# gabrielspmoreira/chameleon_recsys

Hardware: NVIDIA H100
Metric: NAR train interactions/sec (higher is better)
Workload: dtype f32 (wgmma: bf16x3 (error-compensated) forward, single-pass TF32 backward; fp32 accumulate)

## Files before the change

chameleon_recsys_b200/_lib.py:

```python
from __future__ import annotations

import ctypes as C
import os
from typing import Optional

HERE = os.path.dirname(os.path.abspath(__file__))
LIB_PATH = os.path.join(HERE, 'libnar_b200.so')

NAR_MAX_SEGMENTS = 24
NAR_MAX_SRC = 16
NAR_MAX_COLS = 1024

ACT_NONE, ACT_LEAKY, ACT_TANH = 0, 1, 2


class NarError(RuntimeError):
    pass


class Segment(C.Structure):
    _fields_ = [('kind', C.c_int32), ('col', C.c_int32), ('width', C.c_int32), ('card', C.c_int32),
                ('src', C.c_int32), ('ld', C.c_int32), ('table', C.c_void_p), ('grad', C.c_void_p)]


# ... 117 lines not shown
    'nar_dropout_rows': (C.c_int, [vp, vp, i64, i64, i64, vp, i64, i64, i64, C.c_int, f32, u64, u32, vp]),
    'nar_rank_candidates': (C.c_int, [vp, vp, i64, i64, i32, vp, vp, vp, vp]),
    'nar_car_combine_grid': (C.c_int, [vp, vp, i64, i64, i64, C.c_int, vp, vp]),
    'nar_topn_candidates': (C.c_int, [vp, vp, i64, i64, i32, vp, vp, i64, vp, vp, vp, vp]),
    'nar_engine_recommend_workspace_bytes': (C.c_int, [vp, i64, i64, i64, i32, i64, C.POINTER(i64), C.POINTER(i64),
                                                       C.POINTER(i64)]),
    'nar_engine_recommend': (C.c_int, [vp, C.POINTER(StepIO), vp, vp, i64, vp, i64, i32, i32, i64, i64, vp, vp, vp, vp]),
    'nar_host_state_update': (C.c_int, [vp, i64, vp, vp, i64, i64, vp, vp, vp, vp, i64, C.c_double]),
    'nar_host_state_update_batch': (C.c_int, [vp, i64, vp, vp, vp, i64, i64, i64, vp, vp, vp, vp, vp, i64, C.c_double]),
    'nar_state_update': (C.c_int, [vp, vp, i64, vp, vp, i64, i64, i64, vp, vp, vp, vp, vp, vp, i64, C.c_double, vp, vp]),
    'nar_colsum_add': (C.c_int, [vp, i64, i64, i64, vp, vp]),
    'nar_act_bwd': (C.c_int, [vp, vp, i64, C.c_int, vp, vp]),
    'nar_l2_loss_add': (C.c_int, [vp, i64, f32, vp, vp]),
    'nar_transpose_f32': (C.c_int, [vp, i64, i64, i64, vp, i64, vp]),
    'nar_adam_tf': (C.c_int, [vp, vp, vp, vp, i64, i64, f32, f32, f32, f32, f32, i64, vp, vp]),
    'nar_tf32_lo': (C.c_int, [vp, i64, vp, vp]),
    'nar_baselines_clear': (C.c_int, [vp, vp, vp, vp, i64, vp]),
    'nar_baselines_rehash': (C.c_int, [vp, vp, vp, vp, i64, vp, vp, vp, vp, i64, vp, vp]),
    'nar_baselines_update': (C.c_int, [vp, vp, vp, vp, i64, vp, vp, i64, i64, i64, i32, i64, vp, vp]),
    'nar_baselines_buffer_hist': (C.c_int, [vp, i64, i64, vp, vp, vp, vp]),
    'nar_baselines_row_norms': (C.c_int, [vp, i64, i64, i64, vp, vp]),
    'nar_baselines_score': (C.c_int, [vp, vp, vp, vp, i64, vp, vp, vp, i64, i64, i64, vp, vp, vp, vp, i64, i64, vp, i64,
                                      C.c_double, C.c_double, i32, i32, vp, vp, vp, vp, vp]),
    'nar_sknn_update': (C.c_int, [vp, vp, vp, i64, i64, i64, i64, vp, vp, vp, vp, vp, i64, i64, i64, vp, vp]),
    'nar_sknn_score': (C.c_int, [vp, vp, vp, i64, i64, i64, i64, vp, vp, vp, i64, i64, i64, i64, i64, i64, i32, i32, i32,
                                 vp, vp, vp, vp, vp]),
    'nar_eval_metrics_mark': (C.c_int, [vp, i64, i64, i32, vp, vp, vp]),
    'nar_eval_metrics_lists': (C.c_int, [vp, i64, i64, i64, i64, i64, i64, i32, vp, i64, vp, vp, i64, i64, vp, i64,
                                         C.c_double, vp, vp, vp, vp]),
    'nar_eval_metrics_reduce': (C.c_int, [vp, i64, i64, i64, vp, vp]),
# ... 55 lines not shown
```

chameleon_recsys_b200/csrc/engine.cu:

```cuda
#include "common.cuh"
#include <string.h>
#include <stdio.h>
#include <stdlib.h>

extern "C" int nar_sample_negatives_uidx(nar_ctx*, const int64_t*, int64_t, int64_t, int64_t, int64_t, const int64_t*, int64_t,
                                         int64_t, int64_t, uint64_t, uint32_t, int64_t*, int32_t*, const int64_t**,
                                         const int32_t**, void*, int64_t, void*);
namespace nar {
int recommend_rows(const int32_t* pos_idx, int64_t L, const int64_t* item_clicked, const int64_t* cand_ids, int64_t N,
                   int32_t* row_pos, int64_t* row_item, cudaStream_t st);
}

namespace {

constexpr int N_EVENTS = 64;

inline int64_t align_up(int64_t x, int64_t a) { return (x + a - 1) / a * a; }

struct Carver {
  char* base; int64_t off;
  explicit Carver(void* b) : base(static_cast<char*>(b)), off(0) {}
  template <typename T> T* take(int64_t n) {
    T* p = base ? reinterpret_cast<T*>(base + off) : nullptr;
    off = align_up(off + (n > 0 ? n : 1) * (int64_t)sizeof(T), 256);
    return p;
  }
};

struct PrepBufs {
  void* sampler_ws; int64_t sampler_bytes;
  int64_t* neg; int32_t* neg_uidx; float* stats; int32_t* row_pos; int64_t* row_item;
  int32_t* base_pos; int64_t* base_item; int64_t U;
};

struct StepBufs {
  float *X, *dX, *H1, *E, *dE, *dH1, *F1, *PR, *logits, *PD, *dPD, *Z1, *Z2, *Z3, *dZ1, *dZ2, *dZ3, *dPR, *dF1, *dHO;
  float *GX[NAR_MAX_LAYERS], *HO[NAR_MAX_LAYERS], *GT[NAR_MAX_LAYERS], *CD[NAR_MAX_LAYERS], *dGX[NAR_MAX_LAYERS],
        *HPV[NAR_MAX_LAYERS], *dHOb[NAR_MAX_LAYERS], *HOd[NAR_MAX_LAYERS],
        *UO[NAR_MAX_LAYERS], *RH[NAR_MAX_LAYERS];
  float *PP, *PI, *PC, *DB;
  float* H1cT; int64_t ldr;
};

}

constexpr int MAX_PLANES = 32;
struct PlaneSet {
// ... 2 lines not shown
  int64_t dst[MAX_PLANES];
  const float* W[MAX_PLANES]; void* out[MAX_PLANES];
  uint16_t* buf; void* descs;
};

struct nar_engine {
  nar_ctx* ctx;
  nar_model_cfg cfg;
  PlaneSet planes;
  cudaStream_t aux;
  cudaEvent_t ev[N_EVENTS];
  int ev_i;
  float* WhT[NAR_MAX_LAYERS];
  int64_t launches;
  int fused_product;
};

namespace {

bool fused_product(const nar_engine* e) {
  const nar_model_cfg& c = e->cfg;
  return e->fused_product && c.ranking == 0 && c.K + 1 <= 128 && c.fwd_precision == 4 && c.bwd_precision == 1;
}

int64_t gate_blocks(const nar_model_cfg& c) { return c.rnn_cell == NAR_CELL_LSTM ? 4 : c.rnn_cell == NAR_CELL_GRU ? 3 : 2; }

nar_feature_plan call_plan(const nar_model_cfg& c, const nar_step_io* io, const float* stats) {
  nar_feature_plan plan = c.plan;
  for (int i = 0; i < NAR_MAX_SRC; ++i) { plan.ctx_int[i] = io->ctx_int[i]; plan.ctx_float[i] = io->ctx_float[i]; }
  plan.pop_norm = io->pop_norm;
// ... 5 lines not shown
  const nar_model_cfg& c = e->cfg;
  const int64_t K = c.K, n_cand = K + 1, Rcap = L_cap * (n_cand + 1);
  Carver cv(base);
  int64_t sb = 0;
  nar_sample_negatives_workspace(Bg, T + 1, c.buf_len, K, &sb);
  pb->sampler_bytes = sb;
  pb->sampler_ws = cv.take<char>(sb);
  pb->neg = cv.take<int64_t>(Bg * T * K);
  pb->neg_uidx = cv.take<int32_t>(c.dedup ? Bg * T * K : 1);
  pb->stats = cv.take<float>(24);
  pb->row_pos = cv.take<int32_t>(Rcap);
  pb->row_item = cv.take<int64_t>(Rcap);
  pb->U = K * 20 + 1;
  pb->base_pos = cv.take<int32_t>(c.dedup ? 2 * L_cap + pb->U : 1);
  pb->base_item = cv.take<int64_t>(c.dedup ? 2 * L_cap + pb->U : 1);
  (void)B;
  return cv.off;
}

void session_carve(const nar_model_cfg& c, int64_t L, Carver& cv, StepBufs* sb) {
  const int64_t Hp = c.Hp;
  for (int i = 0; i < c.layers; ++i) {
    sb->GX[i] = cv.take<float>(L * gate_blocks(c) * Hp); sb->HO[i] = cv.take<float>(L * Hp);
    if (c.rnn_cell != NAR_CELL_LSTM) sb->GT[i] = cv.take<float>(L * Hp);
    sb->CD[i] = cv.take<float>(L * Hp);
    if (c.rnn_cell == NAR_CELL_GRU) { sb->UO[i] = cv.take<float>(L * Hp); sb->RH[i] = cv.take<float>(L * Hp); }
  }
  sb->F1 = cv.take<float>(L * 512);
  sb->PR = cv.take<float>(L * c.C);
}
// ... 175 lines not shown
  }
  s.fwd(rnn_in, Hp, c.off_W3, 512, c.off_b3, sb.F1, 512, L, 512, Hp, NAR_ACT_LEAKY_RELU, st);
  if (drop) s.dropout(sb.F1, sb.F1, L, 512, io->pos_idx, 4, st);
  s.fwd(sb.F1, 512, c.off_W4, C, c.off_b4, sb.PR, C, L, C, 512, NAR_ACT_TANH, st);
}

int run_step(nar_engine* e, const nar_step_io* io, cudaStream_t main) {
  const nar_model_cfg& c = e->cfg;
  const int64_t B = io->B, T = io->T, L = io->L, K = c.K, n_cand = K + 1, Rc = L * n_cand, R = L + Rc;
  const int64_t C = c.C, Hp = c.Hp, Fp = c.Fp, c0 = c.ctx_col0;
  const int train = io->train;
  if (L > io->L_cap || L < 0 || B <= 0) return NAR_ERR_INVALID;
  PrepBufs pb; StepBufs sb;
  if (prep_carve(e, io->Bg, B, T, io->L_cap, io->prep_ws, &pb) > io->prep_ws_bytes) return NAR_ERR_WORKSPACE;
  if (step_carve(e, io->L_cap, train, io->ws, &sb) > io->ws_bytes) return NAR_ERR_WORKSPACE;
  NAR_CHECK_CUDA(cudaMemsetAsync(io->loss, 0, 4 * sizeof(float), main));
  if (train) NAR_CHECK_CUDA(cudaMemsetAsync(c.grads, 0, (size_t)c.n_params * sizeof(float), main));
  if (L == 0) return NAR_OK;
  const bool drop = train && c.keep_prob < 1.f;
  if (drop && c.dedup) return NAR_ERR_INVALID;
  Seq s(e, io, main);
  const float inv_count = 1.0f / (float)(io->L_global > 0 ? io->L_global : 1);
  const int64_t U = pb.U, NB = 2 * L + U;

  const nar_feature_plan plan = call_plan(c, io, pb.stats);
  nar_row_layout rl;
  if (c.dedup) { rl.n_rows = NB; rl.n_input = L; rl.n_cand = 0; rl.n_positive = L; rl.n_full = 2 * L; rl.ctx_col0 = c0; }
  else { rl.n_rows = R; rl.n_input = L; rl.n_cand = n_cand; rl.n_positive = 0; rl.n_full = R; rl.ctx_col0 = c0; }
  const int32_t* g_pos = c.dedup ? pb.base_pos : pb.row_pos;
  const int64_t* g_item = c.dedup ? pb.base_item : pb.row_item;
  s.chk(nar_gather_features(e->ctx, &plan, g_pos, g_item, &rl, io->event_ts, io->max_ts, sb.X, main));
  if (drop) s.dropout(sb.X, sb.X, R, Fp, pb.row_pos, 0, main);

  float* H1c = sb.H1 + L * C; float* Ec = sb.E + L * C;
  clicked_rows_forward(s, sb, L, drop);
  if (c.dedup) {
    s.fwd(sb.X + L * Fp, Fp, c.off_W1, C, c.off_b1, sb.PP, C, L, C, Fp, NAR_ACT_NONE, main);
    s.fwd(sb.X + 2 * L * Fp, Fp, c.off_W1, C, -1, sb.PI, C, U, C, c0, NAR_ACT_NONE, main);
    s.fwd(sb.X + c0, Fp, c.off_W1 + c0 * C, C, c.off_b1, sb.PC, C, L, C, Fp - c0, NAR_ACT_NONE, main);
    s.chk(nar_car_combine_t(sb.PP, sb.PC, sb.PI, io->pos_idx, pb.neg_uidx, L, K, C, NAR_ACT_LEAKY_RELU, sb.H1cT, sb.ldr, main));
    s.fwd(sb.H1cT, sb.ldr, c.off_W2, C, c.off_b2, Ec, C, Rc, C, C, NAR_ACT_TANH, main, nullptr, 0, 0, 0);
  } else {
    s.fwd(sb.X + L * Fp, Fp, c.off_W1, C, c.off_b1, H1c, C, Rc, C, Fp, NAR_ACT_LEAKY_RELU, main);
    s.fwd(H1c, C, c.off_W2, C, c.off_b2, Ec, C, Rc, C, C, NAR_ACT_TANH, main);
  }
  s.join();

  nar_novelty_reg nov; memset(&nov, 0, sizeof(nov));
  nov.factor = c.novelty_reg_factor; nov.log_base = c.plan.log_base_novelty; nov.pop_norm = io->pop_norm;
  nov.cand_ids = pb.row_item + L; nov.loss_nov = io->loss + 2;
  const nar_novelty_reg* novp = c.novelty_reg_factor > 0.f ? &nov : nullptr;
  const bool fused = fused_product(e);
  s.scorer(Ec, sb.PR, L, n_cand, fused, sb.PD, sb.Z1, sb.Z2, sb.Z3, sb.logits, io->loss, inv_count, train ? sb.dZ3 : nullptr,
           train ? sb.dE + L * C : nullptr, train ? sb.dPR : nullptr, novp);
  if (c.reg_l2 > 0.f && c.rank == 0) { cudaStream_t st = s.fork(); s.chk(nar_l2_loss_add(c.params, c.reg_end, c.reg_l2, io->loss + 1, st)); }
  if (!train || s.rc) { s.join(); return s.rc; }

  float* dEc = sb.dE + L * C;
  if (c.ranking == 0) {
    { cudaStream_t st = s.fork(); s.wgrad(sb.Z2, 64, sb.dZ3, 32, c.off_M[2], c.ld_M[2], 64, 32, Rc, st); s.bgrad(sb.dZ3, 32, Rc, 32, c.off_c[2], st); }
    s.dgrad(sb.dZ3, 32, c.off_M[2], c.ld_M[2], sb.dZ2, 64, Rc, 64, 32, NAR_ACT_LEAKY_RELU, sb.Z2, 64, 0, main);
    { cudaStream_t st = s.fork(); s.wgrad(sb.Z1, 128, sb.dZ2, 64, c.off_M[1], c.ld_M[1], 128, 64, Rc, st); s.bgrad(sb.dZ2, 64, Rc, 64, c.off_c[1], st); }
    s.dgrad(sb.dZ2, 64, c.off_M[1], c.ld_M[1], sb.dZ1, 128, Rc, 128, 64, NAR_ACT_LEAKY_RELU, sb.Z1, 128, 0, main);
    {
      cudaStream_t st = s.fork();
      if (fused) s.wgrad(Ec, C, sb.dZ1, 128, c.off_M[0], c.ld_M[0], C, 128, Rc, st, sb.PR, C, n_cand);
      else s.wgrad(sb.PD, C, sb.dZ1, 128, c.off_M[0], c.ld_M[0], C, 128, Rc, st);
      s.bgrad(sb.dZ1, 128, Rc, 128, c.off_c[0], st);
    }
    if (fused) {
// ... 220 lines not shown
  add(c.off_M[0], C, 128, c.ld_M[0]); add(c.off_M[1], 128, 64, c.ld_M[1]); add(c.off_M[2], 64, 32, c.ld_M[2]);
  for (int i = 0; i < c.layers; ++i) {
    const int64_t gw = gate_blocks(c) * Hp;
    add(c.off_Wx[i], i == 0 ? C : Hp, gw, gw);
  }
  if (overflow) return NAR_ERR_INVALID;
  if (!ps.buf) {
    cudaMalloc(&ps.buf, (size_t)total * sizeof(uint16_t));
    cudaMemset(ps.buf, 0, (size_t)total * sizeof(uint16_t));
    cudaMalloc(&ps.descs, MAX_PLANES * 32);
  }
  for (int i = 0; i < ps.n; ++i) { ps.W[i] = c.params + ps.off_W[i]; ps.out[i] = ps.buf + ps.dst[i]; }
  return NAR_OK;
}

int planes_refresh(nar_engine* e, cudaStream_t st) {
  PlaneSet& ps = e->planes;
  if (!ps.buf || ps.n == 0) return NAR_ERR_INVALID;
  ++e->launches;
  return nar_pack_bf16x3(ps.W, ps.out, ps.K, ps.N, ps.ldw, ps.ld_out, ps.n, ps.descs, st);
}

extern "C" int nar_engine_create(nar_ctx* ctx, const nar_model_cfg* cfg, nar_engine** out) {
  if (!ctx || !cfg || !out) return NAR_ERR_INVALID;
  *out = nullptr;
  if (cfg->layers < 1 || cfg->layers > NAR_MAX_LAYERS || cfg->rnn_cell < NAR_CELL_UGRNN || cfg->rnn_cell > NAR_CELL_LSTM ||
      cfg->ranking < 0 || cfg->ranking > 1)
    return NAR_ERR_UNSUPPORTED;
  if ((cfg->C & 3) || (cfg->Hp & 3) || (cfg->Fp & 3) || (cfg->ctx_col0 & 3) || cfg->ctx_col0 <= 0 || cfg->ctx_col0 >= cfg->Fp)
    return NAR_ERR_INVALID;
  if (!cfg->params || !cfg->grads || !cfg->adam_m || !cfg->adam_v || !cfg->params_lo) return NAR_ERR_INVALID;
  nar_engine* e = new nar_engine();
  memset(e, 0, sizeof(*e));
  e->ctx = ctx; e->cfg = *cfg;
  { const char* v = getenv("NAR_FUSED_SCORER_PRODUCT"); e->fused_product = !(v && atoi(v) == 0); }
  NAR_CHECK_CUDA(cudaSetDevice(ctx->device));
  if (cudaStreamCreateWithFlags(&e->aux, cudaStreamNonBlocking) != cudaSuccess) { delete e; return NAR_ERR_NO_DEVICE; }
  for (int i = 0; i < N_EVENTS; ++i)
    if (cudaEventCreateWithFlags(&e->ev[i], cudaEventDisableTiming) != cudaSuccess) { delete e; return NAR_ERR_NO_DEVICE; }
  for (int i = 0; i < cfg->layers; ++i) {
    const size_t wht = (size_t)gate_blocks(*cfg) * cfg->Hp * cfg->Hp;
    if (cudaMalloc(&e->WhT[i], wht * sizeof(float)) != cudaSuccess) { delete e; return NAR_ERR_NO_DEVICE; }
  }
  if (planes_build(e) != NAR_OK) { delete e; return NAR_ERR_INVALID; }
  if (!e->planes.buf || !e->planes.descs) { delete e; return NAR_ERR_NO_DEVICE; }
  *out = e;
  return NAR_OK;
}

extern "C" int nar_engine_refresh(nar_engine* e, void* stream) {
  if (!e) return NAR_ERR_INVALID;
  return planes_refresh(e, as_stream(stream));
}

extern "C" int nar_engine_destroy(nar_engine* e) {
  if (!e) return NAR_OK;
  cudaStreamSynchronize(e->aux);
  for (int i = 0; i < NAR_MAX_LAYERS; ++i) if (e->WhT[i]) cudaFree(e->WhT[i]);
  for (int i = 0; i < N_EVENTS; ++i) if (e->ev[i]) cudaEventDestroy(e->ev[i]);
  if (e->aux) cudaStreamDestroy(e->aux);
  if (e->planes.buf) cudaFree(e->planes.buf);
  if (e->planes.descs) cudaFree(e->planes.descs);
  delete e;
  return NAR_OK;
}

extern "C" int nar_engine_update_cfg(nar_engine* e, const nar_model_cfg* cfg) {
  if (!e || !cfg) return NAR_ERR_INVALID;
  if (cfg->layers != e->cfg.layers || cfg->Hp != e->cfg.Hp || cfg->C != e->cfg.C || cfg->Fp != e->cfg.Fp ||
      cfg->rnn_cell != e->cfg.rnn_cell) return NAR_ERR_INVALID;
  e->cfg = *cfg;
  return planes_build(e);
}

extern "C" int nar_engine_workspace_bytes(const nar_engine* e, int64_t Bg, int64_t B, int64_t T, int64_t L_cap, int32_t train,
                                          int64_t* prep_bytes, int64_t* ws_bytes) {
  if (!e || Bg <= 0 || B <= 0 || T <= 0 || L_cap < 0) return NAR_ERR_INVALID;
  PrepBufs pb; StepBufs sb;
  if (prep_bytes) *prep_bytes = prep_carve(e, Bg, B, T, L_cap, nullptr, &pb);
  if (ws_bytes) *ws_bytes = step_carve(e, L_cap, train, nullptr, &sb);
  return NAR_OK;
}

extern "C" int nar_engine_prepare(nar_engine* e, const nar_step_io* io, void* stream) {
  if (!e || !io || !io->prep_ws || !io->all_items || !io->buffer) return NAR_ERR_INVALID;
  const nar_model_cfg& c = e->cfg;
  const int64_t B = io->B, Bg = io->Bg, T = io->T, L = io->L, K = c.K, n_cand = K + 1, R = L + L * n_cand;
  if (L > io->L_cap || io->sess0 < 0 || io->sess0 + B > Bg) return NAR_ERR_INVALID;
  PrepBufs pb;
  if (prep_carve(e, Bg, B, T, io->L_cap, io->prep_ws, &pb) > io->prep_ws_bytes) return NAR_ERR_WORKSPACE;
  cudaStream_t st = as_stream(stream);
  int64_t* neg_local = pb.neg + io->sess0 * T * K;
  int32_t* uidx_local = c.dedup ? pb.neg_uidx + io->sess0 * T * K : nullptr;
  const int64_t* uitems = nullptr; const int32_t* n_unique = nullptr;
  int rc = nar_sample_negatives_uidx(e->ctx, io->all_items, Bg, T + 1, io->sess0, B, io->buffer, c.buf_len, K, c.n_from_buffer,
                                     c.sampler_seed, io->sampler_step, neg_local, uidx_local, &uitems, &n_unique, pb.sampler_ws,
                                     pb.sampler_bytes, st);
  e->launches += 2;
  if (rc) return rc;
  if (L <= 0) return NAR_OK;
  rc = nar_build_rows(io->pos_idx, L, io->item_clicked, io->label_next, pb.neg, K, pb.row_pos, pb.row_item, st);
  ++e->launches;
  if (rc) return rc;
  rc = nar_feature_stats(e->ctx, io->buffer, c.buf_len, c.n_norm, c.plan.created_at_ts, io->pop_norm, io->max_ts,
                         c.plan.log_base_recency, c.plan.log_base_novelty, pb.row_pos, pb.row_item, R, L, n_cand, io->event_ts,
                         pb.stats, st);
  ++e->launches;
  if (rc) return rc;
  if (c.dedup) {
    rc = nar_build_base_rows(io->pos_idx, L, io->item_clicked, io->label_next, uitems, n_unique, pb.U, pb.neg_uidx, K, pb.base_pos,
                             pb.base_item, st);
    ++e->launches;
  }
  return rc;
}

extern "C" int nar_engine_step(nar_engine* e, const nar_step_io* io, void* stream) {
  if (!e || !io || !io->prep_ws || !io->ws || !io->loss) return NAR_ERR_INVALID;
  return run_step(e, io, as_stream(stream));
}

extern "C" int nar_engine_apply(nar_engine* e, const nar_step_io* io, void* stream) {
  if (!e || !io) return NAR_ERR_INVALID;
  const nar_model_cfg& c = e->cfg;
  ++e->launches;
  int rc = nar_adam_tf(c.params, c.grads, c.adam_m, c.adam_v, c.n_params, c.reg_end, c.reg_l2, c.lr, c.beta1, c.beta2, c.eps,
                       io->global_step + 1, c.params_lo, stream);
  if (rc == NAR_OK && c.fwd_precision == 4) rc = planes_refresh(e, as_stream(stream));
  return rc;
}

extern "C" int nar_engine_recommend_workspace_bytes(const nar_engine* e, int64_t L, int64_t Q, int64_t N, int32_t gather_q,
                                                    int64_t budget_bytes, int64_t* ws_bytes, int64_t* q_block, int64_t* n_block) {
  if (!e || !ws_bytes || !q_block || !n_block || L <= 0 || Q <= 0 || Q > L || N <= 0) return NAR_ERR_INVALID;
  const int64_t b = rec_plan(e, L, Q, N, gather_q != 0, budget_bytes, q_block, n_block);
  if (b < 0) return NAR_ERR_WORKSPACE;
  *ws_bytes = b;
  return NAR_OK;
}

extern "C" int nar_engine_recommend(nar_engine* e, const nar_step_io* io, const int64_t* q_rows, const int32_t* q_pos, int64_t Q,
                                    const int64_t* cand_ids, int64_t N, int32_t top_n, int32_t exclude_session_clicks,
                                    int64_t q_block, int64_t n_block, int64_t* out_ids, float* out_scores, float* out_probs,
                                    void* stream) {
  if (!e || !io || !io->ws || !q_pos || !cand_ids || !out_ids || !io->buffer || !io->pop_norm || !io->item_clicked) return NAR_ERR_INVALID;
  if (io->train) return NAR_ERR_INVALID;
  return run_recommend(e, io, q_rows, q_pos, Q, cand_ids, N, top_n, exclude_session_clicks, q_block, n_block, out_ids, out_scores,
                       out_probs, as_stream(stream));
}

extern "C" int64_t nar_engine_launch_count(const nar_engine* e) { return e ? e->launches : 0; }

extern "C" int nar_engine_buffer(const nar_engine* e, const nar_step_io* io, const char* name, void** ptr, int64_t* rows, int64_t* ld) {
  if (!e || !io || !name || !ptr) return NAR_ERR_INVALID;
  const nar_model_cfg& c = e->cfg;
  const int64_t L = io->L, K = c.K, n_cand = K + 1, Rc = L * n_cand, R = L + Rc;
  PrepBufs pb; StepBufs sb;
  prep_carve(e, io->Bg, io->B, io->T, io->L_cap, io->prep_ws, &pb);
  step_carve(e, io->L_cap, io->train, io->ws, &sb);
  const int64_t NB = 2 * L + pb.U;
  struct Ent { const char* n; void* p; int64_t r, l; };
  const Ent tab[] = {
      {"neg", pb.neg, io->Bg * io->T, K}, {"neg_uidx", pb.neg_uidx, io->Bg * io->T, K}, {"stats", pb.stats, 1, 24},
      {"row_pos", pb.row_pos, R, 1}, {"row_item", pb.row_item, R, 1}, {"base_pos", pb.base_pos, NB, 1},
      {"base_item", pb.base_item, NB, 1},
      {"X", sb.X, c.dedup ? NB : R, c.Fp}, {"dX", sb.dX, c.dedup ? NB : R, c.Fp}, {"H1", sb.H1, R, c.C}, {"H1cT", sb.H1cT, c.C, sb.ldr}, {"E", sb.E, R, c.C},
      {"dE", sb.dE, R, c.C}, {"dH1", sb.dH1, R, c.C}, {"F1", sb.F1, L, 512}, {"PR", sb.PR, L, c.C},
      {"logits", sb.logits, L, n_cand}, {"PD", sb.PD, Rc, c.C}, {"Z1", sb.Z1, Rc, 128}, {"Z2", sb.Z2, Rc, 64}, {"Z3", sb.Z3, Rc, 32}, {"PP", sb.PP, L, c.C},
      {"PI", sb.PI, pb.U, c.C}, {"PC", sb.PC, L, c.C}, {"DB", sb.DB, 3 * L + pb.U, c.C},
      {"HO0", sb.HO[0], L, c.Hp}, {"HO1", sb.HO[1], L, c.Hp}, {"HO2", sb.HO[2], L, c.Hp}, {"HO3", sb.HO[3], L, c.Hp},
      {"HOd0", sb.HOd[0], L, c.Hp}, {"HOd1", sb.HOd[1], L, c.Hp}, {"HOd2", sb.HOd[2], L, c.Hp}, {"HOd3", sb.HOd[3], L, c.Hp}};
  for (const Ent& t : tab)
    if (strcmp(t.n, name) == 0) {
      *ptr = t.p;
      if (rows) *rows = t.r;
      if (ld) *ld = t.l;
      return t.p ? NAR_OK : NAR_ERR_INVALID;
    }
  return NAR_ERR_INVALID;
}
// ... 1 lines not shown
```

chameleon_recsys_b200/csrc/misc.cu:

```cuda
#include "common.cuh"
#include <stdlib.h>

namespace nar {
namespace misc {

__device__ __forceinline__ float tf32_lo(float x) { return x - __uint_as_float(__float_as_uint(x) & 0xFFFFE000u); }

__global__ void __launch_bounds__(256)
adam_tf_kernel(float4* __restrict__ w, const float4* __restrict__ g, float4* __restrict__ m, float4* __restrict__ v,
               int64_t n4, int64_t reg_end4, float reg_l2, float lr_t, float b1, float b2, float eps, float4* __restrict__ wlo) {
  for (int64_t i = (int64_t)blockIdx.x * blockDim.x + threadIdx.x; i < n4; i += (int64_t)gridDim.x * blockDim.x) {
    float4 wi = w[i], gi = g[i], mi = m[i], vi = v[i];
    const float r = i < reg_end4 ? reg_l2 : 0.f;
#define NAR_ADAM1(c)                                              \
    { const float gg = fmaf(r, wi.c, gi.c);                       \
      mi.c = b1 * mi.c + (1.f - b1) * gg;                         \
      vi.c = b2 * vi.c + (1.f - b2) * gg * gg;                    \
      wi.c -= lr_t * mi.c / (sqrtf(vi.c) + eps); }
    NAR_ADAM1(x) NAR_ADAM1(y) NAR_ADAM1(z) NAR_ADAM1(w)
#undef NAR_ADAM1
    w[i] = wi; m[i] = mi; v[i] = vi;
    if (wlo) wlo[i] = make_float4(tf32_lo(wi.x), tf32_lo(wi.y), tf32_lo(wi.z), tf32_lo(wi.w));
  }
}

__global__ void __launch_bounds__(256)
tf32_lo_kernel(const float* __restrict__ x, int64_t n, float* __restrict__ lo) {
  for (int64_t i = (int64_t)blockIdx.x * blockDim.x + threadIdx.x; i < n; i += (int64_t)gridDim.x * blockDim.x) lo[i] = tf32_lo(x[i]);
}

__global__ void __launch_bounds__(256)
colsum_add_kernel(const float* __restrict__ x, int64_t rows, int64_t cols, int64_t ld, float* __restrict__ out) {
  const int64_t c = (int64_t)blockIdx.x * 256 + threadIdx.x;
  const int64_t r0 = (int64_t)blockIdx.y * 64, r1 = min(rows, r0 + 64);
  if (c >= cols) return;
  float a[8] = {0.f, 0.f, 0.f, 0.f, 0.f, 0.f, 0.f, 0.f};
  int64_t r = r0;
// ... 129 lines not shown

extern "C" int nar_ctx_destroy(nar_ctx* ctx) {
  if (ctx) { cudaFree(ctx->gather_desc); free(ctx->gather_key); }
  delete ctx;
  return NAR_OK;
}

extern "C" int nar_tf32_lo(const float* x, int64_t n, float* lo, void* stream) {
  if (!x || !lo) return NAR_ERR_INVALID;
  if (n <= 0) return NAR_OK;
  nar::misc::tf32_lo_kernel<<<nar::misc::grid_for(n, 1024), 256, 0, as_stream(stream)>>>(x, n, lo);
  NAR_LAUNCH_CHECK();
  return NAR_OK;
}

extern "C" int nar_adam_tf(float* params, const float* grads, float* m, float* v, int64_t n, int64_t reg_end, float reg_l2,
                           float lr, float beta1, float beta2, float eps, int64_t step, float* params_lo, void* stream) {
  if (!params || !grads || !m || !v || (n & 3) || (reg_end & 3) || step < 1) return NAR_ERR_INVALID;
  if (n == 0) return NAR_OK;
  const double lr_t = (double)lr * sqrt(1.0 - pow((double)beta2, (double)step)) / (1.0 - pow((double)beta1, (double)step));
  nar::misc::adam_tf_kernel<<<nar::misc::grid_for(n / 4, 256), 256, 0, as_stream(stream)>>>(
      reinterpret_cast<float4*>(params), reinterpret_cast<const float4*>(grads), reinterpret_cast<float4*>(m),
      reinterpret_cast<float4*>(v), n / 4, reg_end / 4, reg_l2, (float)lr_t, beta1, beta2, eps,
      reinterpret_cast<float4*>(params_lo));
  NAR_LAUNCH_CHECK();
  return NAR_OK;
}

extern "C" int nar_dropout_rows(const float* src, float* dst, int64_t rows, int64_t cols, int64_t ld, const int32_t* row_pos,
                                int64_t n_input, int64_t n_cand, int64_t K, int tensor_id, float keep_prob, uint64_t seed,
                                uint32_t step, void* stream) {
  if (!src || !dst || !row_pos || (cols & 3) || (ld & 3) || tensor_id < 0 || tensor_id > 255) return NAR_ERR_INVALID;
  if (!(keep_prob > 0.f) || keep_prob > 1.f) return NAR_ERR_INVALID;
  if (tensor_id == 0 && (n_cand <= 0 || K != n_cand - 1)) return NAR_ERR_INVALID;
  if (rows <= 0 || cols <= 0) return NAR_OK;
  const unsigned long long thr = (unsigned long long)floor((double)keep_prob * 4294967296.0);
  nar::misc::dropout_rows_kernel<<<nar::misc::grid_for(rows * (cols / 4), 256), 256, 0, as_stream(stream)>>>(
      src, dst, rows, (int)(cols / 4), ld, row_pos, n_input, n_cand, K, tensor_id, 1.0f / keep_prob, thr, (uint32_t)seed,
      (uint32_t)(seed >> 32) ^ 0x5DEECE66u, step);
  NAR_LAUNCH_CHECK();
  return NAR_OK;
// ... 37 lines not shown
```

chameleon_recsys_b200/engine.py:

```python
from __future__ import annotations

import ctypes as C
import os
from typing import Dict, Optional

import numpy as np
import torch

from . import ops
from ._lib import FeaturePlanC, ModelCfg, NarError, StepIO, check
from .dp import shard_sessions
from .plan import (SEG_ACR, SEG_CTX_EMBED, SEG_ITEM_EMB, SEG_META_EMBED, FeaturePlan, ParamLayout, round_up)

_NP2T = {np.int64: torch.int64, np.float32: torch.float32, np.int32: torch.int32}


def set_plan_columns(p: FeaturePlanC, pl: FeaturePlan):
    if pl.Fp > len(p.col_seg):
        raise NarError('feature rows wider than NAR_MAX_COLS')
    cs = np.full(len(p.col_seg), 255, dtype=np.uint8)
    wide = np.zeros(pl.Fp, dtype=bool)
    for i, s in enumerate(pl.segments):
        cs[s.int_col:s.int_col + s.width] = i
        if s.kind in (SEG_ACR, SEG_ITEM_EMB):
# ... 393 lines not shown
        cur = torch.cuda.current_stream()
        run_on = stream if stream is not None else cur
        io = self._make_io(st, slot, step_id)
        last_use = self._slot_events.get(slot) if stream is not None else None
        if last_use is not None:
            run_on.wait_event(last_use)
        check(self._lib.nar_engine_prepare(self._handle, C.byref(io), C.c_void_p(run_on.cuda_stream)), 'nar_engine_prepare')
        ev = None
        if stream is not None:
            ev = torch.cuda.Event()
            ev.record(run_on)
        st['prep'] = {'io': io, 'event': ev, 'step_id': step_id, 'slot': slot}
        return st

    _INT_BUFFERS = {'neg': torch.int64, 'row_item': torch.int64, 'base_item': torch.int64, 'neg_uidx': torch.int32,
                    'row_pos': torch.int32, 'base_pos': torch.int32}

    def buffer(self, st: dict, name: str) -> torch.Tensor:
        io = st['prep']['io']
        ptr, rows, ld = C.c_void_p(), C.c_int64(0), C.c_int64(0)
        check(self._lib.nar_engine_buffer(self._handle, C.byref(io), name.encode(), C.byref(ptr), C.byref(rows), C.byref(ld)),
              'nar_engine_buffer(%s)' % name)
        dt = self._INT_BUFFERS.get(name, torch.float32)
        esz = torch.empty((), dtype=dt).element_size()
        for owner in st['_hold']:
            o = ptr.value - owner.data_ptr()
            if 0 <= o < owner.numel():
                n = rows.value * ld.value
                return owner[o:o + n * esz].view(dt).view(rows.value, ld.value)
        raise NarError('buffer %s is outside the step workspaces' % name)

# ... 226 lines not shown
```

chameleon_recsys_b200/ops.py:

```python
from __future__ import annotations

import ctypes as C
from typing import Optional

import torch

from . import _lib
from ._lib import ACT_LEAKY, ACT_NONE, ACT_TANH, Context, FeaturePlanC, GemmEpilogue, NarError, check

_ctx: dict = {}
LAUNCHES = 0


def context(device: Optional[int] = None) -> Context:
    if device is None:
        device = torch.cuda.current_device()
    if device not in _ctx:
        _ctx[device] = Context(device)
    return _ctx[device]


_STREAM_OVERRIDE: Optional[int] = None


# ... 288 lines not shown


def transpose(src, rows, cols, ld_src, dst, ld_dst):
    global LAUNCHES
    LAUNCHES += 1
    check(_lib.load().nar_transpose_f32(_p(src), rows, cols, ld_src, _p(dst), ld_dst, _stream()), 'nar_transpose_f32')


def adam_tf(params, grads, m, v, n, reg_end, reg_l2, lr, step, beta1=0.9, beta2=0.999, eps=1e-8, params_lo=None):
    global LAUNCHES
    LAUNCHES += 1
    check(_lib.load().nar_adam_tf(_p(params), _p(grads), _p(m), _p(v), n, reg_end, reg_l2, lr, beta1, beta2, eps, step,
                                  _p(params_lo), _stream()), 'nar_adam_tf')


def tf32_lo(x, n, lo):
    global LAUNCHES
    LAUNCHES += 1
    check(_lib.load().nar_tf32_lo(_p(x), n, _p(lo), _stream()), 'nar_tf32_lo')
```

include/nar_b200.h:

```cpp
#ifndef NAR_B200_H
#define NAR_B200_H

#include <stdint.h>

#ifdef __cplusplus
extern "C" {
#endif

#define NAR_ABI_VERSION 3

typedef enum {
  NAR_OK = 0,
  NAR_ERR_INVALID = -1,
  NAR_ERR_UNSUPPORTED = -2,
  NAR_ERR_NO_DEVICE = -3,
  NAR_ERR_WORKSPACE = -4
} nar_status;

typedef struct nar_ctx nar_ctx;

int  nar_abi_version(void);
int  nar_abi_struct_size(int which);
const char* nar_status_string(int status);
int  nar_ctx_create(int device, nar_ctx** out);
// ... 197 lines not shown
                     int64_t* new_ts, int64_t* recent_pop, float* pop_norm, double* pop_norm64, int64_t* articles_pop,
                     int64_t num_items, double min_norm_pop, int* err, void* stream);

int nar_dropout_rows(const float* src, float* dst, int64_t rows, int64_t cols, int64_t ld, const int32_t* row_pos,
                     int64_t n_input, int64_t n_cand, int64_t K, int tensor_id, float keep_prob, uint64_t seed,
                     uint32_t step, void* stream);

int nar_colsum_add(const float* x, int64_t rows, int64_t cols, int64_t ld, float* out, void* stream);
int nar_act_bwd(const float* dy, const float* y, int64_t n, int act, float* dx, void* stream);
int nar_l2_loss_add(const float* x, int64_t n, float scale, float* out, void* stream);
int nar_transpose_f32(const float* src, int64_t rows, int64_t cols, int64_t ld_src, float* dst, int64_t ld_dst, void* stream);

int nar_adam_tf(float* params, const float* grads, float* m, float* v, int64_t n, int64_t reg_end,
                float reg_l2, float lr, float beta1, float beta2, float eps, int64_t step,
                float* params_lo , void* stream);
int nar_tf32_lo(const float* x, int64_t n, float* lo, void* stream);

#define NAR_MAX_LAYERS 4

typedef struct {
  int64_t num_items, C , Hp , Fp , ctx_col0;
  int32_t layers, rnn_cell , ranking ;
  int32_t fwd_precision, bwd_precision;
  int32_t dedup;
  int32_t use_aux_stream;
  float keep_prob;
  float novelty_reg_factor;
  uint64_t dropout_seed;
  int64_t K , n_from_buffer, buf_len, n_norm;
  float inv_temperature, reg_l2, lr, beta1, beta2, eps;
// ... 101 lines not shown
```

Baseline: 302,600.

## Split Adam over item-embedding rows and overlap untouched-row updates with forward

Before each step, the prep stage marks which item-embedding rows the batch touches. Gradient zeroing then clears only rows touched in the previous or next step instead of memsetting the whole gradient buffer. The Adam update for rows with zero gradient runs on a forked stream during the forward pass. The apply step then updates only the touched rows plus all non-embedding parameters. This cuts the serial full-parameter memory traffic on the critical path, at the cost of new state bookkeeping (double-buffered row masks, pending-update event) and the need for exact consistency with the Adam semantics.

```diff
diff --git a/chameleon_recsys_b200/_lib.py b/chameleon_recsys_b200/_lib.py
--- a/chameleon_recsys_b200/_lib.py
+++ b/chameleon_recsys_b200/_lib.py
@@ -155,6 +155,7 @@
     'nar_l2_loss_add': (C.c_int, [vp, i64, f32, vp, vp]),
     'nar_transpose_f32': (C.c_int, [vp, i64, i64, i64, vp, i64, vp]),
     'nar_adam_tf': (C.c_int, [vp, vp, vp, vp, i64, i64, f32, f32, f32, f32, f32, i64, vp, vp]),
+    'nar_adam_tf_rows': (C.c_int, [vp, vp, vp, vp, i64, i64, f32, f32, f32, f32, f32, i64, vp, vp, i64, i64, i64, i32, vp]),
     'nar_tf32_lo': (C.c_int, [vp, i64, vp, vp]),
     'nar_baselines_clear': (C.c_int, [vp, vp, vp, vp, i64, vp]),
     'nar_baselines_rehash': (C.c_int, [vp, vp, vp, vp, i64, vp, vp, vp, vp, i64, vp, vp]),
diff --git a/chameleon_recsys_b200/csrc/engine.cu b/chameleon_recsys_b200/csrc/engine.cu
--- a/chameleon_recsys_b200/csrc/engine.cu
+++ b/chameleon_recsys_b200/csrc/engine.cu
@@ -9,6 +9,10 @@
 namespace nar {
 int recommend_rows(const int32_t* pos_idx, int64_t L, const int64_t* item_clicked, const int64_t* cand_ids, int64_t N,
                    int32_t* row_pos, int64_t* row_item, cudaStream_t st);
+int grad_zero_rows(float* grads, int64_t n, int64_t row_off, int64_t n_rows, int64_t ld, const uint8_t* prev, const uint8_t* next,
+                   uint8_t* keep, cudaStream_t st);
+int rows_mark(const int64_t* a, int64_t na, const int64_t* b, int64_t nb, const int64_t* u, const int32_t* nu, int64_t n_rows,
+              uint8_t* rows, cudaStream_t st);
 }
 
 namespace {
@@ -31,6 +35,7 @@
   void* sampler_ws; int64_t sampler_bytes;
   int64_t* neg; int32_t* neg_uidx; float* stats; int32_t* row_pos; int64_t* row_item;
   int32_t* base_pos; int64_t* base_item; int64_t U;
+  uint8_t* rows;
 };
 
 struct StepBufs {
@@ -63,6 +68,12 @@
   float* WhT[NAR_MAX_LAYERS];
   int64_t launches;
   int fused_product;
+  int64_t emb_off, emb_rows, emb_ld;
+  uint8_t* rows[2]; int rows_cur;
+  bool upd_armed;
+  bool upd_pending;
+  int64_t upd_step;
+  cudaEvent_t upd_ev;
 };
 
 namespace {
@@ -98,6 +109,7 @@
   pb->U = K * 20 + 1;
   pb->base_pos = cv.take<int32_t>(c.dedup ? 2 * L_cap + pb->U : 1);
   pb->base_item = cv.take<int64_t>(c.dedup ? 2 * L_cap + pb->U : 1);
+  pb->rows = e->emb_rows ? cv.take<uint8_t>(e->emb_rows) : nullptr;
   (void)B;
   return cv.off;
 }
@@ -303,8 +315,23 @@
   PrepBufs pb; StepBufs sb;
   if (prep_carve(e, io->Bg, B, T, io->L_cap, io->prep_ws, &pb) > io->prep_ws_bytes) return NAR_ERR_WORKSPACE;
   if (step_carve(e, io->L_cap, train, io->ws, &sb) > io->ws_bytes) return NAR_ERR_WORKSPACE;
+  if (e->upd_pending) return NAR_ERR_INVALID;
   NAR_CHECK_CUDA(cudaMemsetAsync(io->loss, 0, 4 * sizeof(float), main));
-  if (train) NAR_CHECK_CUDA(cudaMemsetAsync(c.grads, 0, (size_t)c.n_params * sizeof(float), main));
+  bool upd = false;
+  if (train) {
+    if (e->emb_rows) {
+      uint8_t* keep = e->rows[e->rows_cur ^ 1];
+      const int rc = nar::grad_zero_rows(c.grads, c.n_params, e->emb_off, e->emb_rows, e->emb_ld, e->rows[e->rows_cur], pb.rows,
+                                         keep, main);
+      ++e->launches;
+      if (rc) return rc;
+      e->rows_cur ^= 1;
+      upd = e->upd_armed && L > 0;
+    } else {
+      NAR_CHECK_CUDA(cudaMemsetAsync(c.grads, 0, (size_t)c.n_params * sizeof(float), main));
+    }
+    e->upd_armed = false;
+  }
   if (L == 0) return NAR_OK;
   const bool drop = train && c.keep_prob < 1.f;
   if (drop && c.dedup) return NAR_ERR_INVALID;
@@ -320,6 +347,13 @@
   const int64_t* g_item = c.dedup ? pb.base_item : pb.row_item;
   s.chk(nar_gather_features(e->ctx, &plan, g_pos, g_item, &rl, io->event_ts, io->max_ts, sb.X, main));
   if (drop) s.dropout(sb.X, sb.X, R, Fp, pb.row_pos, 0, main);
+  if (c.reg_l2 > 0.f && c.rank == 0) { cudaStream_t st = s.fork(); s.chk(nar_l2_loss_add(c.params, c.reg_end, c.reg_l2, io->loss + 1, st)); }
+  if (upd && !s.rc) {
+    cudaStream_t st = s.fork();
+    s.chk(nar_adam_tf_rows(c.params, nullptr, c.adam_m, c.adam_v, c.n_params, c.reg_end, c.reg_l2, c.lr, c.beta1, c.beta2, c.eps,
+                           io->global_step + 1, c.params_lo, e->rows[e->rows_cur], e->emb_off, e->emb_rows, e->emb_ld, 1, st));
+    if (!s.rc && cudaEventRecord(e->upd_ev, st) == cudaSuccess) { e->upd_pending = true; e->upd_step = io->global_step + 1; }
+  }
 
   float* H1c = sb.H1 + L * C; float* Ec = sb.E + L * C;
   clicked_rows_forward(s, sb, L, drop);
@@ -342,7 +376,6 @@
   const bool fused = fused_product(e);
   s.scorer(Ec, sb.PR, L, n_cand, fused, sb.PD, sb.Z1, sb.Z2, sb.Z3, sb.logits, io->loss, inv_count, train ? sb.dZ3 : nullptr,
            train ? sb.dE + L * C : nullptr, train ? sb.dPR : nullptr, novp);
-  if (c.reg_l2 > 0.f && c.rank == 0) { cudaStream_t st = s.fork(); s.chk(nar_l2_loss_add(c.params, c.reg_end, c.reg_l2, io->loss + 1, st)); }
   if (!train || s.rc) { s.join(); return s.rc; }
 
   float* dEc = sb.dE + L * C;
@@ -593,6 +626,29 @@
   return NAR_OK;
 }
 
+int emb_setup(nar_engine* e) {
+  const nar_model_cfg& c = e->cfg;
+  int64_t off = 0, rows = 0, ld = 0;
+  for (int i = 0; i < c.plan.n_segments; ++i) {
+    const nar_segment& sg = c.plan.seg[i];
+    if (sg.kind != NAR_SEG_ITEM_EMB || !sg.table) continue;
+    off = sg.table - c.params; rows = sg.card; ld = sg.ld;
+    if (sg.grad != c.grads + off || off < 0 || (off & 3) || ld <= 0 || (ld & 3) || rows <= 0 || off + rows * ld > c.n_params ||
+        rows * ld / 4 > 0xFFFFFFFFll)
+      rows = 0;
+  }
+  if (rows == e->emb_rows && (rows == 0 || (off == e->emb_off && ld == e->emb_ld))) return NAR_OK;
+  for (uint8_t*& r : e->rows) { if (r) cudaFree(r); r = nullptr; }
+  e->emb_off = off; e->emb_rows = rows; e->emb_ld = ld; e->rows_cur = 0;
+  e->upd_armed = e->upd_pending = false;
+  for (uint8_t*& r : e->rows) {
+    if (rows == 0) break;
+    NAR_CHECK_CUDA(cudaMalloc(&r, (size_t)rows));
+    NAR_CHECK_CUDA(cudaMemset(r, 1, (size_t)rows));
+  }
+  return NAR_OK;
+}
+
 int planes_refresh(nar_engine* e, cudaStream_t st) {
   PlaneSet& ps = e->planes;
   if (!ps.buf || ps.n == 0) return NAR_ERR_INVALID;
@@ -623,6 +679,9 @@
   }
   if (planes_build(e) != NAR_OK) { delete e; return NAR_ERR_INVALID; }
   if (!e->planes.buf || !e->planes.descs) { delete e; return NAR_ERR_NO_DEVICE; }
+  if (cudaEventCreateWithFlags(&e->upd_ev, cudaEventDisableTiming) != cudaSuccess || emb_setup(e) != NAR_OK) {
+    delete e; return NAR_ERR_NO_DEVICE;
+  }
   *out = e;
   return NAR_OK;
 }
@@ -640,6 +699,8 @@
   if (e->aux) cudaStreamDestroy(e->aux);
   if (e->planes.buf) cudaFree(e->planes.buf);
   if (e->planes.descs) cudaFree(e->planes.descs);
+  for (uint8_t* r : e->rows) if (r) cudaFree(r);
+  if (e->upd_ev) cudaEventDestroy(e->upd_ev);
   delete e;
   return NAR_OK;
 }
@@ -649,7 +710,8 @@
   if (cfg->layers != e->cfg.layers || cfg->Hp != e->cfg.Hp || cfg->C != e->cfg.C || cfg->Fp != e->cfg.Fp ||
       cfg->rnn_cell != e->cfg.rnn_cell) return NAR_ERR_INVALID;
   e->cfg = *cfg;
-  return planes_build(e);
+  const int rc = emb_setup(e);
+  return rc ? rc : planes_build(e);
 }
 
 extern "C" int nar_engine_workspace_bytes(const nar_engine* e, int64_t Bg, int64_t B, int64_t T, int64_t L_cap, int32_t train,
@@ -677,6 +739,12 @@
                                      pb.sampler_bytes, st);
   e->launches += 2;
   if (rc) return rc;
+  if (e->emb_rows) {
+    rc = nar::rows_mark(io->all_items, Bg * (T + 1), io->label_next, io->label_next ? Bg * T : 0, uitems, n_unique, e->emb_rows,
+                        pb.rows, st);
+    ++e->launches;
+    if (rc) return rc;
+  }
   if (L <= 0) return NAR_OK;
   rc = nar_build_rows(io->pos_idx, L, io->item_clicked, io->label_next, pb.neg, K, pb.row_pos, pb.row_item, st);
   ++e->launches;
@@ -702,9 +770,20 @@
 extern "C" int nar_engine_apply(nar_engine* e, const nar_step_io* io, void* stream) {
   if (!e || !io) return NAR_ERR_INVALID;
   const nar_model_cfg& c = e->cfg;
+  const int64_t t = io->global_step + 1;
   ++e->launches;
-  int rc = nar_adam_tf(c.params, c.grads, c.adam_m, c.adam_v, c.n_params, c.reg_end, c.reg_l2, c.lr, c.beta1, c.beta2, c.eps,
-                       io->global_step + 1, c.params_lo, stream);
+  int rc;
+  if (e->upd_pending) {
+    if (t != e->upd_step) return NAR_ERR_INVALID;
+    NAR_CHECK_CUDA(cudaStreamWaitEvent(as_stream(stream), e->upd_ev, 0));
+    rc = nar_adam_tf_rows(c.params, c.grads, c.adam_m, c.adam_v, c.n_params, c.reg_end, c.reg_l2, c.lr, c.beta1, c.beta2, c.eps, t,
+                          c.params_lo, e->rows[e->rows_cur], e->emb_off, e->emb_rows, e->emb_ld, 0, stream);
+    e->upd_pending = false;
+  } else {
+    rc = nar_adam_tf(c.params, c.grads, c.adam_m, c.adam_v, c.n_params, c.reg_end, c.reg_l2, c.lr, c.beta1, c.beta2, c.eps, t,
+                     c.params_lo, stream);
+  }
+  if (rc == NAR_OK) e->upd_armed = true;
   if (rc == NAR_OK && c.fwd_precision == 4) rc = planes_refresh(e, as_stream(stream));
   return rc;
 }
@@ -723,7 +802,7 @@
                                     int64_t q_block, int64_t n_block, int64_t* out_ids, float* out_scores, float* out_probs,
                                     void* stream) {
   if (!e || !io || !io->ws || !q_pos || !cand_ids || !out_ids || !io->buffer || !io->pop_norm || !io->item_clicked) return NAR_ERR_INVALID;
-  if (io->train) return NAR_ERR_INVALID;
+  if (io->train || e->upd_pending) return NAR_ERR_INVALID;
   return run_recommend(e, io, q_rows, q_pos, Q, cand_ids, N, top_n, exclude_session_clicks, q_block, n_block, out_ids, out_scores,
                        out_probs, as_stream(stream));
 }
@@ -742,7 +821,7 @@
   const Ent tab[] = {
       {"neg", pb.neg, io->Bg * io->T, K}, {"neg_uidx", pb.neg_uidx, io->Bg * io->T, K}, {"stats", pb.stats, 1, 24},
       {"row_pos", pb.row_pos, R, 1}, {"row_item", pb.row_item, R, 1}, {"base_pos", pb.base_pos, NB, 1},
-      {"base_item", pb.base_item, NB, 1},
+      {"base_item", pb.base_item, NB, 1}, {"rows", pb.rows, e->emb_rows, 1},
       {"X", sb.X, c.dedup ? NB : R, c.Fp}, {"dX", sb.dX, c.dedup ? NB : R, c.Fp}, {"H1", sb.H1, R, c.C}, {"H1cT", sb.H1cT, c.C, sb.ldr}, {"E", sb.E, R, c.C},
       {"dE", sb.dE, R, c.C}, {"dH1", sb.dH1, R, c.C}, {"F1", sb.F1, L, 512}, {"PR", sb.PR, L, c.C},
       {"logits", sb.logits, L, n_cand}, {"PD", sb.PD, Rc, c.C}, {"Z1", sb.Z1, Rc, 128}, {"Z2", sb.Z2, Rc, 64}, {"Z3", sb.Z3, Rc, 32}, {"PP", sb.PP, L, c.C},
diff --git a/chameleon_recsys_b200/csrc/misc.cu b/chameleon_recsys_b200/csrc/misc.cu
--- a/chameleon_recsys_b200/csrc/misc.cu
+++ b/chameleon_recsys_b200/csrc/misc.cu
@@ -6,11 +6,21 @@
 
 __device__ __forceinline__ float tf32_lo(float x) { return x - __uint_as_float(__float_as_uint(x) & 0xFFFFE000u); }
 
+enum { ADAM_ALL = 0, ADAM_TAIL = 1, ADAM_UNTOUCHED = 2 };
+
+template <int PASS>
 __global__ void __launch_bounds__(256)
 adam_tf_kernel(float4* __restrict__ w, const float4* __restrict__ g, float4* __restrict__ m, float4* __restrict__ v,
-               int64_t n4, int64_t reg_end4, float reg_l2, float lr_t, float b1, float b2, float eps, float4* __restrict__ wlo) {
-  for (int64_t i = (int64_t)blockIdx.x * blockDim.x + threadIdx.x; i < n4; i += (int64_t)gridDim.x * blockDim.x) {
-    float4 wi = w[i], gi = g[i], mi = m[i], vi = v[i];
+               int64_t n4, int64_t reg_end4, float reg_l2, float lr_t, float b1, float b2, float eps, float4* __restrict__ wlo,
+               const uint8_t* __restrict__ rows, int64_t row0_4, uint32_t block4, uint32_t ld4) {
+  const int64_t lo = PASS == ADAM_UNTOUCHED ? row0_4 : 0, hi = PASS == ADAM_UNTOUCHED ? row0_4 + block4 : n4;
+  for (int64_t i = lo + (int64_t)blockIdx.x * blockDim.x + threadIdx.x; i < hi; i += (int64_t)gridDim.x * blockDim.x) {
+    if (PASS != ADAM_ALL) {
+      const uint64_t e = (uint64_t)(i - row0_4);
+      if (e < block4 && (rows[(uint32_t)e / ld4] != 0) != (PASS == ADAM_TAIL)) continue;
+    }
+    float4 wi = w[i], mi = m[i], vi = v[i];
+    const float4 gi = PASS == ADAM_UNTOUCHED ? make_float4(0.f, 0.f, 0.f, 0.f) : g[i];
     const float r = i < reg_end4 ? reg_l2 : 0.f;
 #define NAR_ADAM1(c)                                              \
     { const float gg = fmaf(r, wi.c, gi.c);                       \
@@ -21,6 +31,30 @@
 #undef NAR_ADAM1
     w[i] = wi; m[i] = mi; v[i] = vi;
     if (wlo) wlo[i] = make_float4(tf32_lo(wi.x), tf32_lo(wi.y), tf32_lo(wi.z), tf32_lo(wi.w));
+  }
+}
+
+__global__ void __launch_bounds__(256)
+grad_zero_rows_kernel(float4* __restrict__ g, int64_t n4, int64_t row0_4, uint32_t block4, uint32_t ld4,
+                      const uint8_t* __restrict__ prev, const uint8_t* __restrict__ next, uint8_t* __restrict__ keep) {
+  for (int64_t i = (int64_t)blockIdx.x * blockDim.x + threadIdx.x; i < n4; i += (int64_t)gridDim.x * blockDim.x) {
+    const uint64_t e = (uint64_t)(i - row0_4);
+    if (e < block4) {
+      const uint32_t row = (uint32_t)e / ld4;
+      if ((uint32_t)e == row * ld4) keep[row] = next[row];
+      if (!(prev[row] | next[row])) continue;
+    }
+    g[i] = make_float4(0.f, 0.f, 0.f, 0.f);
+  }
+}
+
+__global__ void __launch_bounds__(256)
+rows_mark_kernel(const int64_t* __restrict__ a, int64_t na, const int64_t* __restrict__ b, int64_t nb,
+                 const int64_t* __restrict__ u, const int32_t* __restrict__ nu, int64_t n_rows, uint8_t* __restrict__ rows) {
+  const int64_t nu_ = u ? *nu : 0, n = na + nb + nu_;
+  for (int64_t i = (int64_t)blockIdx.x * blockDim.x + threadIdx.x; i <= n; i += (int64_t)gridDim.x * blockDim.x) {
+    const int64_t id = i == n ? 0 : i < na ? a[i] : i < na + nb ? b[i - na] : u[i - na - nb];
+    if (id >= 0 && id < n_rows) rows[id] = 1;
   }
 }
 
@@ -180,17 +214,61 @@
   return NAR_OK;
 }
 
+static float adam_lr_t(float lr, float beta1, float beta2, int64_t step) {
+  return (float)((double)lr * sqrt(1.0 - pow((double)beta2, (double)step)) / (1.0 - pow((double)beta1, (double)step)));
+}
+
 extern "C" int nar_adam_tf(float* params, const float* grads, float* m, float* v, int64_t n, int64_t reg_end, float reg_l2,
                            float lr, float beta1, float beta2, float eps, int64_t step, float* params_lo, void* stream) {
   if (!params || !grads || !m || !v || (n & 3) || (reg_end & 3) || step < 1) return NAR_ERR_INVALID;
   if (n == 0) return NAR_OK;
-  const double lr_t = (double)lr * sqrt(1.0 - pow((double)beta2, (double)step)) / (1.0 - pow((double)beta1, (double)step));
-  nar::misc::adam_tf_kernel<<<nar::misc::grid_for(n / 4, 256), 256, 0, as_stream(stream)>>>(
+  nar::misc::adam_tf_kernel<nar::misc::ADAM_ALL><<<nar::misc::grid_for(n / 4, 256), 256, 0, as_stream(stream)>>>(
       reinterpret_cast<float4*>(params), reinterpret_cast<const float4*>(grads), reinterpret_cast<float4*>(m),
-      reinterpret_cast<float4*>(v), n / 4, reg_end / 4, reg_l2, (float)lr_t, beta1, beta2, eps,
-      reinterpret_cast<float4*>(params_lo));
-  NAR_LAUNCH_CHECK();
-  return NAR_OK;
+      reinterpret_cast<float4*>(v), n / 4, reg_end / 4, reg_l2, adam_lr_t(lr, beta1, beta2, step), beta1, beta2, eps,
+      reinterpret_cast<float4*>(params_lo), nullptr, 0, 0, 1);
+  NAR_LAUNCH_CHECK();
+  return NAR_OK;
+}
+
+extern "C" int nar_adam_tf_rows(float* params, const float* grads, float* m, float* v, int64_t n, int64_t reg_end, float reg_l2,
+                                float lr, float beta1, float beta2, float eps, int64_t step, float* params_lo, const uint8_t* rows,
+                                int64_t row_off, int64_t n_rows, int64_t ld, int32_t untouched, void* stream) {
+  using namespace nar::misc;
+  if (!params || (!grads && !untouched) || !m || !v || !rows || (n & 3) || (reg_end & 3) || step < 1) return NAR_ERR_INVALID;
+  if ((row_off & 3) || (ld & 3) || ld <= 0 || n_rows <= 0 || row_off < 0 || row_off + n_rows * ld > n) return NAR_ERR_INVALID;
+  if (n_rows * ld / 4 > 0xFFFFFFFFll) return NAR_ERR_UNSUPPORTED;
+  const uint32_t block4 = (uint32_t)(n_rows * ld / 4), ld4 = (uint32_t)(ld / 4);
+  const float lr_t = adam_lr_t(lr, beta1, beta2, step);
+  float4 *w4 = reinterpret_cast<float4*>(params), *m4 = reinterpret_cast<float4*>(m), *v4 = reinterpret_cast<float4*>(v);
+  float4* lo4 = reinterpret_cast<float4*>(params_lo);
+  if (untouched)
+    adam_tf_kernel<ADAM_UNTOUCHED><<<NAR_GRID_SMS * 2, 256, 0, as_stream(stream)>>>(
+        w4, nullptr, m4, v4, n / 4, reg_end / 4, reg_l2, lr_t, beta1, beta2, eps, lo4, rows, row_off / 4, block4, ld4);
+  else
+    adam_tf_kernel<ADAM_TAIL><<<grid_for(n / 4, 256), 256, 0, as_stream(stream)>>>(
+        w4, reinterpret_cast<const float4*>(grads), m4, v4, n / 4, reg_end / 4, reg_l2, lr_t, beta1, beta2, eps, lo4, rows,
+        row_off / 4, block4, ld4);
+  NAR_LAUNCH_CHECK();
+  return NAR_OK;
+}
+
+namespace nar {
+int grad_zero_rows(float* grads, int64_t n, int64_t row_off, int64_t n_rows, int64_t ld, const uint8_t* prev, const uint8_t* next,
+                   uint8_t* keep, cudaStream_t st) {
+  using namespace nar::misc;
+  grad_zero_rows_kernel<<<grid_for(n / 4, 256), 256, 0, st>>>(reinterpret_cast<float4*>(grads), n / 4, row_off / 4,
+                                                             (uint32_t)(n_rows * ld / 4), (uint32_t)(ld / 4), prev, next, keep);
+  NAR_LAUNCH_CHECK();
+  return NAR_OK;
+}
+
+int rows_mark(const int64_t* a, int64_t na, const int64_t* b, int64_t nb, const int64_t* u, const int32_t* nu, int64_t n_rows,
+              uint8_t* rows, cudaStream_t st) {
+  NAR_CHECK_CUDA(cudaMemsetAsync(rows, 0, (size_t)n_rows, st));
+  nar::misc::rows_mark_kernel<<<nar::misc::grid_for(na + nb + 1024, 256), 256, 0, st>>>(a, na, b, nb, u, nu, n_rows, rows);
+  NAR_LAUNCH_CHECK();
+  return NAR_OK;
+}
 }
 
 extern "C" int nar_dropout_rows(const float* src, float* dst, int64_t rows, int64_t cols, int64_t ld, const int32_t* row_pos,
diff --git a/chameleon_recsys_b200/engine.py b/chameleon_recsys_b200/engine.py
--- a/chameleon_recsys_b200/engine.py
+++ b/chameleon_recsys_b200/engine.py
@@ -431,7 +431,7 @@
         return st
 
     _INT_BUFFERS = {'neg': torch.int64, 'row_item': torch.int64, 'base_item': torch.int64, 'neg_uidx': torch.int32,
-                    'row_pos': torch.int32, 'base_pos': torch.int32}
+                    'row_pos': torch.int32, 'base_pos': torch.int32, 'rows': torch.uint8}
 
     def buffer(self, st: dict, name: str) -> torch.Tensor:
         io = st['prep']['io']
diff --git a/chameleon_recsys_b200/ops.py b/chameleon_recsys_b200/ops.py
--- a/chameleon_recsys_b200/ops.py
+++ b/chameleon_recsys_b200/ops.py
@@ -326,6 +326,15 @@
                                   _p(params_lo), _stream()), 'nar_adam_tf')
 
 
+def adam_tf_rows(params, grads, m, v, n, reg_end, reg_l2, lr, step, rows, row_off, n_rows, ld, untouched, beta1=0.9,
+                 beta2=0.999, eps=1e-8, params_lo=None):
+    global LAUNCHES
+    LAUNCHES += 1
+    check(_lib.load().nar_adam_tf_rows(_p(params), _p(grads), _p(m), _p(v), n, reg_end, reg_l2, lr, beta1, beta2, eps, step,
+                                       _p(params_lo), _p(rows), row_off, n_rows, ld, int(bool(untouched)), _stream()),
+          'nar_adam_tf_rows')
+
+
 def tf32_lo(x, n, lo):
     global LAUNCHES
     LAUNCHES += 1
diff --git a/include/nar_b200.h b/include/nar_b200.h
--- a/include/nar_b200.h
+++ b/include/nar_b200.h
@@ -235,6 +235,9 @@
 int nar_adam_tf(float* params, const float* grads, float* m, float* v, int64_t n, int64_t reg_end,
                 float reg_l2, float lr, float beta1, float beta2, float eps, int64_t step,
                 float* params_lo , void* stream);
+int nar_adam_tf_rows(float* params, const float* grads, float* m, float* v, int64_t n, int64_t reg_end, float reg_l2,
+                     float lr, float beta1, float beta2, float eps, int64_t step, float* params_lo, const uint8_t* rows,
+                     int64_t row_off, int64_t n_rows, int64_t ld, int32_t untouched, void* stream);
 int nar_tf32_lo(const float* x, int64_t n, float* lo, void* stream);
 
 #define NAR_MAX_LAYERS 4
```

Measured after the change: 306,900, median of 6. +1.4%, better.
